# cambyse/po-rrt

Hardware: AMD Instinct MI355X
Metric: RRT node-expansions/sec on map_benchmark.pgm (higher is better)
Workload: dtype f64

## Files before the change

### po_rrt_amd/csrc/porrt_device.hpp

```cpp
#pragma once
#include <hip/hip_runtime.h>
#include <stdint.h>
#include <string>
#include <vector>
#include "../../include/porrt_hip.h"

namespace porrt {

template <int NEV>
struct ScopedEvents {
    hipEvent_t e[NEV];
    ScopedEvents() { for (int i = 0; i < NEV; ++i) e[i] = nullptr; }
    hipError_t create() {
        for (int i = 0; i < NEV; ++i) { const hipError_t r = hipEventCreate(&e[i]); if (r != hipSuccess) return r; }
        return hipSuccess;
    }
    ~ScopedEvents() { for (int i = 0; i < NEV; ++i) if (e[i]) (void)hipEventDestroy(e[i]); }
    ScopedEvents(const ScopedEvents &) = delete;
    ScopedEvents &operator=(const ScopedEvents &) = delete;
};

template <class Launch, class GoingOn>
static int sweep_to_fixpoint(hipStream_t stream, uint32_t *flags, size_t rows, int cur, Launch &&launch, GoingOn &&going_on, const char *who,
                             uint64_t &sweeps, std::string &err) {
// ... 619 lines not shown
        if (m < INF) break;
    }
    if (m == INF && !PTO) m = dist2(rc.nx[0], rc.ny[0], qx, qy);
    return m;
}

__device__ __forceinline__ uint32_t rank_before(const RunConst &rc, uint32_t b, uint32_t vwords, uint32_t k);
__device__ __forceinline__ uint32_t wave_sum(uint32_t v);
__device__ void commit_rrt_sample(const RunConst &rc, uint32_t b, uint32_t vwords, uint32_t k, uint32_t lane, uint32_t stride = 64u, bool lag = false);
constexpr int kRG = 40;
constexpr uint32_t kRegions = kRG * kRG;
constexpr uint32_t kPage = 64;
constexpr uint32_t kOccWords = (kRegions + 63u) / 64u;
typedef double dbl2 __attribute__((ext_vector_type(2)));

__device__ __forceinline__ uint32_t region_of(const RunConst &rc, double x, double y) {
    int cx, cy;
    rep_cell(rc, x, y, kRG, cx, cy);
    return (uint32_t)(cy * kRG + cx);
}

__device__ __forceinline__ double disc_radius(double bound_d2, double qx, double qy) {
    return sqrt(bound_d2) * (1.0 + 1e-9) + 1e-12 * (1.0 + fabs(qx) + fabs(qy));
}

template <class Visit>
__device__ __forceinline__ void scan_disc(const RunConst &rc, uint32_t b, double qx, double qy, double rho, uint32_t N, uint32_t lane, Visit visit,
                                          uint32_t skip_region = 0xFFFFFFFFu, uint32_t share = 0u, uint32_t nshare = 1u) {
    int cx0, cy0, cx1, cy1;
    rep_cell(rc, qx - rho, qy - rho, kRG, cx0, cy0);
    rep_cell(rc, qx + rho, qy + rho, kRG, cx1, cy1);
    const uint32_t x0 = uni((uint32_t)cx0), y0 = uni((uint32_t)cy0);
    const uint32_t w = uni((uint32_t)(cx1 - cx0 + 1)), nreg = w * uni((uint32_t)(cy1 - cy0 + 1));
    if (nreg * 16u > N) {
        auto gx = as_global(rc.nx), gy = as_global(rc.ny);
        for (uint32_t j0 = share * 128u; j0 < N; j0 += nshare * 128u) {
            double x[2], y[2];
#pragma unroll
            for (int u = 0; u < 2; ++u) {
                const uint32_t j = j0 + 64u * u + lane;
                x[u] = gx[j < N ? j : 0u];
                y[u] = gy[j < N ? j : 0u];
            }
#pragma unroll
            for (int u = 0; u < 2; ++u)
                if (j0 + 64u * u < N) visit(x[u], y[u], (int)(j0 + 64u * u + lane), j0 + 64u * u + lane < N);
        }
        return;
    }
    auto gcnt = as_global(rc.rg_cnt) + (b & 1u) * kRegions;
    auto gdir = as_global(rc.rg_dir);
    auto gxy = as_global(reinterpret_cast<const dbl2 *>(rc.pg_xy));
    auto gid = as_global(rc.pg_id);
    for (uint32_t r0 = 0; r0 < nreg; r0 += 64) {
        const uint32_t r = r0 + lane;
        uint32_t reg = 0, cnt = 0;
        if (r < nreg) {
            const uint32_t ry = r / w;
            reg = (y0 + ry) * kRG + x0 + (r - ry * w);
            cnt = reg == skip_region ? 0u : gcnt[reg];
        }
        const uint32_t npg = (uint32_t)__popcll(__ballot(cnt > 0u));
        if (__ballot(cnt >= npg || cnt > kPage) == 0ull && npg > 1u) {
            if (nshare > 1u && r % nshare != share) cnt = 0u;
            uint32_t cmax = cnt;
            for (int off = 32; off > 0; off >>= 1) {
                const uint32_t o = __shfl_xor(cmax, off);
                cmax = o > cmax ? o : cmax;
            }
            cmax = uni(cmax);
            for (uint32_t s0 = 0; s0 < cmax; s0 += 2) {
                dbl2 v[2];
                int id[2];
#pragma unroll
                for (int u = 0; u < 2; ++u) {
                    const uint32_t sl = s0 + u < cnt ? s0 + u : 0u;
                    v[u] = gxy[(size_t)reg * kPage + sl];
                    id[u] = gid[(size_t)reg * kPage + sl];
                }
#pragma unroll
                for (int u = 0; u < 2; ++u)
                    if (s0 + u < cmax) visit(v[u].x, v[u].y, id[u], s0 + u < cnt);
            }
            continue;
        }
        uint32_t page = reg;
        for (uint32_t j = 0;; ++j) {
            unsigned long long m = __ballot(cnt > j * kPage);
            if (!m) break;
            if (nshare > 1u) m = __ballot(cnt > j * kPage && (r + j) % nshare == share);
            if (j && cnt > j * kPage) page = gdir[(size_t)reg * rc.rg_maxp + j];
            while (m) {
                uint32_t pg[2], pc[2];
#pragma unroll
                for (int u = 0; u < 2; ++u) {
                    pg[u] = 0; pc[u] = 0;
                    if (m) {
                        const uint32_t l = (uint32_t)__builtin_ctzll(m);
                        m &= m - 1;
                        pg[u] = (uint32_t)__builtin_amdgcn_readlane((int)page, (int)l);
                        const uint32_t c = (uint32_t)__builtin_amdgcn_readlane((int)cnt, (int)l) - j * kPage;
                        pc[u] = c < kPage ? c : kPage;
                    }
                }
                dbl2 v[2];
                int id[2];
#pragma unroll
                for (int u = 0; u < 2; ++u) {
                    const bool ld = lane < pc[u];
                    v[u] = ld ? gxy[(size_t)pg[u] * kPage + lane] : dbl2{0.0, 0.0};
                    id[u] = ld ? gid[(size_t)pg[u] * kPage + lane] : -1;
                }
#pragma unroll
                for (int u = 0; u < 2; ++u)
                    if (pc[u]) visit(v[u].x, v[u].y, id[u], lane < pc[u]);
            }
        }
    }
}

template <bool PTO>
__device__ __forceinline__ void near_sample(const RunConst &rc, uint32_t b, uint32_t i0, uint32_t vwords, uint32_t k, uint32_t lane) {
    const uint32_t N = uni(as_global(rc.n_at)[b]);
    const double sqx = uni_d(as_global(rc.sx)[i0 + k]), sqy = uni_d(as_global(rc.sy)[i0 + k]);
    uint32_t world = 0;
    if (PTO) world = uni(as_global(rc.sworld)[i0 + k]);
    const double INF = __longlong_as_double(0x7FF0000000000000ll);
// ... 550 lines not shown
    GlobalList L;
    L.cid = as_global((const int *)rc.cand_id) + cand_off(rc, b, k);
    L.cxy = as_global(reinterpret_cast<const dbl2 *>(rc.cand_xy)) + cand_off(rc, b, k);
    L.cval = as_global(rc.cand_val) + cand_val_off(rc, b, k);
    L.gdA = as_global((const double *)rc.distA);
    return L;
}
#ifndef PORRT_LDS_HITS
#define PORRT_LDS_HITS 80
#endif
constexpr uint32_t kLdsHits = PORRT_LDS_HITS;
static_assert(kLdsHits % 2u == 0u, "kLdsHits");
constexpr uint32_t kHitBytes = kLdsHits * (4u + 8u + 8u + 8u);
struct LdsHits {
    static constexpr bool kCompact = true;
    int *hid;
    double *hx, *hy, *hd;
    GPTR(int) out_id;
    GPTR(double) out_val;
    GPTR(uint32_t) out_cnt;
    uint32_t out_cap;
    __device__ __forceinline__ int id(uint32_t a) const { return hid[a]; }
    __device__ __forceinline__ void xy(uint32_t a, double &x, double &y) const { x = hx[a]; y = hy[a]; }
    __device__ __forceinline__ double val(uint32_t a) const { return hx[a]; }
    __device__ __forceinline__ void set_val(uint32_t a, double v) const { hx[a] = v; }
    __device__ __forceinline__ void set_dA(uint32_t, double) const {}
    __device__ __forceinline__ double dA(uint32_t a, int) const { return hd[a]; }
};
struct MemHits {
    static constexpr bool kCompact = true;
    GPTR(int) sid;
    GPTR(dbl2) sxy;
    GPTR(double) sd;
    GPTR(int) out_id;
    GPTR(double) out_val;
    GPTR(uint32_t) out_cnt;
    uint32_t out_cap;
    __device__ __forceinline__ int id(uint32_t a) const { return sid[a]; }
    __device__ __forceinline__ void xy(uint32_t a, double &x, double &y) const { const dbl2 v = sxy[a]; x = v.x; y = v.y; }
    __device__ __forceinline__ double val(uint32_t a) const { return sxy[a].x; }
    __device__ __forceinline__ void set_val(uint32_t a, double v) const { sxy[a].x = v; }
    __device__ __forceinline__ void set_dA(uint32_t, double) const {}
    __device__ __forceinline__ double dA(uint32_t a, int) const { return sd[a]; }
};

struct NoNearestSearch { __device__ int operator()() const { return 0; } };
template <class TeamT, class ListT, class Grid, class NNF = NoNearestSearch>
__device__ void connect_rrt_sample(const RunConst &rc, const TeamT &tm, const ListT &L, const Grid &grid, uint32_t b, uint32_t k, uint32_t id,
                                   double px, double py, uint32_t cnt, uint32_t &err, const uint32_t *clone_ids = nullptr, uint32_t n_clone = 0,
                                   int clr_known = -1, NNF nearest_search = NNF(), uint32_t swap = 0) {
// ... 238 lines not shown
    }
    PORRT_TACC_S(rc, 6);
    auto gdB = as_global(reinterpret_cast<unsigned long long *>(swap ? rc.distA : rc.distB));
    if constexpr (ListT::kCompact) {
        {
            uint32_t n_out = 0;
            for (uint32_t a0 = 0; a0 < cnt; a0 += TS) {
                const uint32_t a = a0 + tl;
                double via = -1.0;
                int j = -1;
                if (a < cnt) {
                    const double cost = a0 == 0 ? cost0 : L.val(a);
                    j = a0 == 0 ? j0 : L.id(a);
                    if (nvalid != 0 && cost >= 0.0 && j != best) {
                        const double v = dnew + cost;
                        if (v < (a0 == 0 ? dA0 : L.dA(a, j))) { g_atomic_min(gdB + j, f64_bits(v)); via = v; }
                    }
                }
                const unsigned long long hm = tm.ballot(via >= 0.0);
                const uint32_t pos = n_out + (uint32_t)__popcll(hm & ((1ull << tm.sub()) - 1ull));
                if (via >= 0.0) {
                    if (pos < L.out_cap) { L.out_id[pos] = j; L.out_val[pos] = via; }
                    else err |= ERR_CAND_OVERFLOW;
                }
                n_out += (uint32_t)__popcll(hm);
            }
            if (tl == 0) *L.out_cnt = n_out;
        }
        PORRT_TACC_S(rc, 7);
        return;
    } else {
// ... 1587 lines not shown
```

### po_rrt_amd/csrc/porrt_engine.hip

```cpp
#include "../../include/porrt_hip.h"
#include "porrt_host.hpp"
#include "porrt_device.hpp"
#include "porrt_group.hpp"
#include "porrt_belief.hpp"
#include "porrt_dp.hpp"
#include "porrt_prm.hpp"
#include "porrt_edges.hpp"
#include "porrt_refine.hpp"
#include "porrt_refine_batch.hpp"
#include "porrt_reparent.hpp"
#include "porrt_qmdp.hpp"
#include "porrt_policy_graph.hpp"
#include "porrt_join.hpp"
#include "porrt_mm_recipe.hpp"

#include <algorithm>
#include <functional>
#include <chrono>
#include <cmath>
#include <cstdio>
#include <cstring>
#include <string>
#include <system_error>
#include <mutex>
// ... 1089 lines not shown
    const uint64_t Nmax = n_iter_max + 2;
    const uint64_t steps_max = n_iter_max / K + 4;
    const uint32_t vwords = (K + 63) / 64;
    const uint32_t Kpad = vwords * 64;
    const uint32_t cand_cap = (uint32_t)std::min<uint64_t>(std::max<uint32_t>(opt_cand_cap, 64), Nmax);
    const uint64_t pend_cap = n_iter_max + 2, pool_cap = tie_pool_ids ? tie_pool_ids : std::max<uint64_t>(1u << 20, tie_pool_mult * n_iter_max);
    {
        double t0 = now_s();
        HIPCHK(d_nx.reserve(Nmax)); HIPCHK(d_ny.reserve(Nmax)); HIPCHK(d_distA.reserve(Nmax)); HIPCHK(d_distB.reserve(Nmax));
        HIPCHK(d_parent.reserve(Nmax)); HIPCHK(d_reachA.reserve(Nmax)); HIPCHK(d_reachB.reserve(Nmax));
        HIPCHK(d_vid.reserve(Nmax)); HIPCHK(d_finalflag.reserve(Nmax + 8)); HIPCHK(d_finalmask.reserve(Nmax));
        HIPCHK(d_nat.reserve(steps_max + 2)); HIPCHK(d_validmask.reserve((steps_max + 2) * vwords));
        HIPCHK(d_sx.reserve(n_iter_max + 1)); HIPCHK(d_sy.reserve(n_iter_max + 1)); HIPCHK(d_sworld.reserve(n_iter_max + 1));
        HIPCHK(d_qx.reserve(2 * Kpad)); HIPCHK(d_qy.reserve(2 * Kpad)); HIPCHK(d_qnn.reserve(2 * Kpad)); HIPCHK(d_qvid.reserve(2 * Kpad));
        const uint64_t rg_maxp = Nmax / kPage + 2, pg_cap = 2ull * kRegions + Nmax / kPage + 8;
        HIPCHK(d_rgcnt.reserve(2 * kRegions)); HIPCHK(d_rgocc.reserve(2 * kOccWords)); HIPCHK(d_rgdir.reserve((size_t)kRegions * rg_maxp));
        HIPCHK(d_pgxy.reserve(2 * (size_t)pg_cap * kPage)); HIPCHK(d_pgid.reserve((size_t)pg_cap * kPage)); HIPCHK(d_pgd.reserve((size_t)pg_cap * kPage)); HIPCHK(d_slotof.reserve(Nmax));
        HIPCHK(d_candcnt.reserve(3 * (size_t)K)); HIPCHK(d_kdbox.reserve(Nmax)); HIPCHK(d_kdlosers.reserve(kClaimMax)); HIPCHK(d_bcscratch.reserve(8 * Nmax + 4096)); HIPCHK(d_bcout.reserve(1)); HIPCHK(d_bccursor.reserve(1)); HIPCHK(d_locbox.reserve(2 * (8 * (size_t)K + 4096))); HIPCHK(d_kdhint.reserve((size_t)kHG * kHG));
        HIPCHK(d_loccur.reserve(2 * (8 * (size_t)K + 4096))); HIPCHK(d_locdcur.reserve(2 * (8 * (size_t)K + 4096))); HIPCHK(d_locgex.reserve(2 * (8 * (size_t)K + 4096))); HIPCHK(d_locflags.reserve(2 * (8 * (size_t)K + 4096)));
        HIPCHK(d_gsnap.reserve((steps_max + 4) * 4)); HIPCHK(d_pendoff.reserve(pend_cap)); HIPCHK(d_pendn.reserve(pend_cap)); HIPCHK(d_pendcur.reserve(pend_cap));
        HIPCHK(d_pendstate.reserve(pend_cap)); HIPCHK(d_pendnew.reserve(pend_cap)); HIPCHK(d_pendpool.reserve(pool_cap)); HIPCHK(d_kdsurv.reserve(Nmax)); HIPCHK(d_gndx.reserve(Nmax)); HIPCHK(d_gndy.reserve(Nmax)); HIPCHK(d_gndbox.reserve(Nmax));
        HIPCHK(d_kqx.reserve((steps_max + 2) * Kpad)); HIPCHK(d_kqy.reserve((steps_max + 2) * Kpad)); HIPCHK(d_kqvid.reserve((steps_max + 2) * Kpad)); { const size_t np = (opt_pipeline == 4 && stage != 1 && K <= 1024) ? 3u : 2u; HIPCHK(d_candid.reserve(np * (size_t)K * cand_cap)); HIPCHK(d_candxy.reserve(2 * np * (size_t)K * cand_cap)); HIPCHK(d_candval.reserve((np == 3u ? 3u : 1u) * (size_t)K * cand_cap)); }
        HIPCHK(d_gid.reserve(Nmax));
        HIPCHK(d_perm.reserve((steps_max + 2) * Kpad)); HIPCHK(d_ssx.reserve((steps_max + 2) * Kpad)); HIPCHK(d_ssy.reserve((steps_max + 2) * Kpad));
        HIPCHK(d_bqx.reserve(Kpad)); HIPCHK(d_bqy.reserve(Kpad)); HIPCHK(d_bqk.reserve(Kpad)); HIPCHK(d_t2at.reserve(steps_max + 4));
        HIPCHK(d_rep.reserve(kRepInts));
        HIPCHK(d_sched_i0.reserve(steps_max + 4)); HIPCHK(d_sched_nb.reserve(steps_max + 4));
        HIPCHK(d_kdrec.reserve(Nmax)); HIPCHK(d_gx.reserve(Nmax + 16)); HIPCHK(d_gy.reserve(Nmax + 16)); HIPCHK(d_kdup.reserve(Nmax)); HIPCHK(d_kddepth.reserve(Nmax)); HIPCHK(d_kdgexit.reserve(Nmax));
        HIPCHK(d_radT2.reserve(Nmax + 8));
        HIPCHK(d_cnt.reserve(1)); HIPCHK(d_rc.reserve(1)); HIPCHK(d_jump.reserve(1));
        if (mode == PORRT_MODE_PTO) {
            const uint64_t ecap = std::min<uint64_t>(Nmax * edge_per_node + 4096, 1ull << 31);
            HIPCHK(d_efrom.reserve(ecap)); HIPCHK(d_eto.reserve(ecap)); HIPCHK(d_etv.reserve(ecap));
        }
        if (has_grid) HIPCHK(d_cls.reserve(cls_bytes(W, H)));
        if (has_inj) HIPCHK(d_inj.reserve(inj_xy.size() + 2));
        int r = layout_buffers();
// ... 3742 lines not shown
```

### po_rrt_amd/csrc/porrt_group.hpp

```cpp
#pragma once
#include "porrt_device.hpp"
#include "porrt_span.hpp"

namespace porrt {


template <int GL, int R, bool WITHD, class Visit>
__device__ __forceinline__ void gscan_disc(const RunConst &rc, uint32_t b, const GTeam<GL> &tm, double qx, double qy, double rho, uint32_t N, Visit visit,
                                           uint32_t skip_region = 0xFFFFFFFFu) {
    const uint32_t gl = tm.gl;
    int cx0, cy0, cx1, cy1;
    rep_cell(rc, qx - rho, qy - rho, kRG, cx0, cy0);
    rep_cell(rc, qx + rho, qy + rho, kRG, cx1, cy1);
    const uint32_t x0 = (uint32_t)cx0, y0 = (uint32_t)cy0;
    const uint32_t w = (uint32_t)(cx1 - cx0 + 1), nreg = w * (uint32_t)(cy1 - cy0 + 1);
    constexpr int U = (int)kPage / GL;
    if (nreg * 16u > N) {
        auto gx = as_global(rc.nx), gy = as_global(rc.ny), gdA = as_global(rc.distA);
        for (uint32_t j0 = 0; j0 < N; j0 += (uint32_t)(U * GL)) {
            double x[U], y[U], d[U];
#pragma unroll
            for (int u = 0; u < U; ++u) {
                const uint32_t j = j0 + (uint32_t)(GL * u) + gl;
                x[u] = gx[j < N ? j : 0u];
                y[u] = gy[j < N ? j : 0u];
                d[u] = WITHD ? gdA[j < N ? j : 0u] : 0.0;
            }
#pragma unroll
            for (int u = 0; u < U; ++u)
                if (j0 + (uint32_t)(GL * u) < N) visit(x[u], y[u], d[u], (int)(j0 + (uint32_t)(GL * u) + gl), j0 + (uint32_t)(GL * u) + gl < N);
        }
        return;
    }
    auto gcnt = as_global(rc.rg_cnt) + (b & 1u) * kRegions;
    auto gdir = as_global(rc.rg_dir);
    auto gxy = as_global(reinterpret_cast<const dbl2 *>(rc.pg_xy));
    auto gid = as_global(rc.pg_id);
    auto gpd = as_global(rc.pg_d);
    for (uint32_t r0 = 0; r0 < nreg; r0 += (uint32_t)GL) {
        const uint32_t r = r0 + gl;
        uint32_t reg = 0, cnt = 0;
        if (r < nreg) {
            const uint32_t ry = r / w;
            reg = (y0 + ry) * kRG + x0 + (r - ry * w);
            cnt = reg == skip_region ? 0u : gcnt[reg];
        }
        uint32_t page = reg;
        for (uint32_t lvl = 0;; ++lvl) {
            const uint32_t have = cnt > lvl * kPage ? cnt - lvl * kPage : 0u;
            unsigned long long m = tm.ballot(have > 0u);
            if (!m) break;
            uint32_t page_next = 0;
            if (have > kPage) page_next = gdir[(size_t)reg * rc.rg_maxp + lvl + 1u];
// ... 7 lines not shown
                        m &= m - 1;
                        pg[q] = tm.shfl(page, l);
                        const uint32_t h = tm.shfl(have, l);
                        pc[q] = h < kPage ? h : kPage;
                    }
                }
                dbl2 v[R][U];
                double d[R][U];
                int id[R][U];
#pragma unroll
                for (int q = 0; q < R; ++q)
#pragma unroll
                    for (int u = 0; u < U; ++u) {
                        const uint32_t sl = (uint32_t)(u * GL) + gl;
                        const bool ld = sl < pc[q];
                        v[q][u] = ld ? gxy[(size_t)pg[q] * kPage + sl] : dbl2{0.0, 0.0};
                        id[q][u] = ld ? gid[(size_t)pg[q] * kPage + sl] : -1;
                        d[q][u] = (WITHD && ld) ? gpd[(size_t)pg[q] * kPage + sl] : 0.0;
                    }
#pragma unroll
                for (int q = 0; q < R; ++q)
#pragma unroll
                    for (int u = 0; u < U; ++u)
                        if ((uint32_t)(u * GL) < pc[q]) visit(v[q][u].x, v[q][u].y, d[q][u], id[q][u], (uint32_t)(u * GL) + gl < pc[q]);
            }
            page = page_next;
        }
    }
}

__device__ __forceinline__ void xcd_swizzle(uint32_t &bx, uint32_t &by) {
    const uint32_t gx = gridDim.x, Q = gridDim.y;
    if (Q & 7u) return;
    const uint32_t L = by * gx + bx, slot = L >> 3;
// ... 85 lines not shown
            }
            m = tm.shfl(d2, 0);
        }
        if (m < INF) break;
    }
    if (m == INF) m = dist2(as_global(rc.nx)[0], as_global(rc.ny)[0], qx, qy);
    return m;
}

#ifndef PORRT_REG_PAGES
#define PORRT_REG_PAGES 1
#endif
template <int GL, class Visit>
__device__ __forceinline__ void gscan_region(const RunConst &rc, const GTeam<GL> &tm, uint32_t reg, uint32_t cnt, Visit visit) {
    auto gdir = as_global(rc.rg_dir);
    auto gxy = as_global(reinterpret_cast<const dbl2 *>(rc.pg_xy));
    auto gid = as_global(rc.pg_id);
    constexpr int U = (int)kPage / GL, RP = PORRT_REG_PAGES;
    const uint32_t npages = (cnt + kPage - 1u) / kPage;
    for (uint32_t j0 = 0; j0 < npages; j0 += (uint32_t)RP) {
        uint32_t page[RP], pc[RP];
#pragma unroll
        for (int q = 0; q < RP; ++q) {
            const uint32_t j = j0 + (uint32_t)q;
            page[q] = 0; pc[q] = 0;
            if (j < npages) {
                page[q] = j ? gdir[(size_t)reg * rc.rg_maxp + j] : reg;
                pc[q] = cnt - j * kPage < kPage ? cnt - j * kPage : kPage;
            }
        }
        dbl2 v[RP][U];
        int id[RP][U];
#pragma unroll
        for (int q = 0; q < RP; ++q)
#pragma unroll
            for (int u = 0; u < U; ++u) {
                const uint32_t sl = (uint32_t)(u * GL) + tm.gl;
                const bool ld = sl < pc[q];
                v[q][u] = ld ? gxy[(size_t)page[q] * kPage + sl] : dbl2{0.0, 0.0};
                id[q][u] = ld ? gid[(size_t)page[q] * kPage + sl] : -1;
            }
#pragma unroll
        for (int q = 0; q < RP; ++q)
#pragma unroll
            for (int u = 0; u < U; ++u)
                if ((uint32_t)(u * GL) < pc[q]) visit(v[q][u].x, v[q][u].y, id[q][u], (uint32_t)(u * GL) + tm.gl < pc[q]);
    }
}

__device__ __forceinline__ double region_gap2(const RunConst &rc, double qx, double qy, int cx, int cy, double wx, double wy) {
    const double INF = __longlong_as_double(0x7FF0000000000000ll);
    const double xlo = cx == 0 ? -INF : rc.bx0 + (double)cx * wx, xhi = cx == kRG - 1 ? INF : rc.bx0 + (double)(cx + 1) * wx;
    const double ylo = cy == 0 ? -INF : rc.by0 + (double)cy * wy, yhi = cy == kRG - 1 ? INF : rc.by0 + (double)(cy + 1) * wy;
    double gx = qx < xlo ? xlo - qx : (qx > xhi ? qx - xhi : 0.0), gy = qy < ylo ? ylo - qy : (qy > yhi ? qy - yhi : 0.0);
    const double eps = 1e-9 * (1.0 + fabs(qx) + fabs(qy));
    gx = gx > eps ? gx - eps : 0.0;
// ... 169 lines not shown
#pragma unroll
        for (uint32_t u = 0; u < kSpanPer; ++u) {
            const uint32_t t = tid * kSpanPer + u, k = k0 + t;
            const uint32_t stored = k < limit ? as_global(rc.cand_cnt)[cand_cnt_at(rc, cb, k)] : 0u;
            c[u] = span_count(stored, cap, span_valid(words, t), k, limit);
            s += c[u];
        }
        uint32_t incl = s;
#pragma unroll
        for (uint32_t off = 1; off < 64u; off <<= 1) {
            const uint32_t v = (uint32_t)__shfl_up((int)incl, off);
            if (tid >= off) incl += v;
        }
        span_prefix_lane(s_prefix, tid, c, incl - s);
    }
    auto gdA = as_global(rc.distA);
    auto gpd = as_global(rc.pg_d);
    auto gso = as_global(rc.slot_of);
    for (uint32_t t = tid; t < kSpan; t += T)
        if (k0 + t < limit && span_valid(words, t)) {
            const uint32_t id = base + span_rank_in(words, t);
            gpd[gso[id]] = gdA[id];
        }
    __syncthreads();
    const uint32_t total = s_prefix[kSpan];
    auto gcid = as_global(rc.cand_id);
    auto gcval = as_global(rc.cand_val);
    auto gdB = as_global(rc.distB);
    constexpr int U = 4;
    for (uint32_t r0 = tid; r0 < total; r0 += T * (uint32_t)U) {
        double via[U], dB[U];
        int j[U], id[U];
#pragma unroll
        for (int u = 0; u < U; ++u) {
            const uint32_t r = r0 + (uint32_t)u * T;
            via[u] = -1.0; j[u] = 0; id[u] = 0;
            if (r < total) {
                const uint32_t t = span_find(s_prefix, r), a = r - s_prefix[t];
                via[u] = gcval[cand_val_off(rc, cb, k0 + t) + a];
                j[u] = gcid[cand_off(rc, cb, k0 + t) + a];
                id[u] = (int)(base + span_rank_in(words, t));
            }
        }
#pragma unroll
        for (int u = 0; u < U; ++u) dB[u] = via[u] >= 0.0 ? gdB[j[u]] : 0.0;
#pragma unroll
        for (int u = 0; u < U; ++u) {
            if (!(via[u] >= 0.0) || f64_bits(via[u]) != f64_bits(dB[u])) continue;
            auto gpar = as_global(rc.parent) + j[u];
            int old = *gpar;
            while (old < N || id[u] < old) {
                int expect = old;
                if (__hip_atomic_compare_exchange_strong(gpar, &expect, id[u], __ATOMIC_RELAXED, __ATOMIC_RELAXED, __HIP_MEMORY_SCOPE_AGENT)) break;
                old = expect;
            }
            gdA[j[u]] = via[u];
            gpd[gso[j[u]]] = via[u];
        }
    }
}

#ifndef PORRT_NN2_WAVES
#define PORRT_NN2_WAVES 5
#endif
template <int GL, int WV = 4>
__global__ __launch_bounds__(WV * 64) __attribute__((amdgpu_waves_per_eu(PORRT_NN2_WAVES, 8))) void k_nn2(const RunConst *__restrict__ rcp, uint32_t b, uint32_t i0, uint32_t nb, uint32_t vwords, uint32_t cb,
                                             uint32_t cnb, uint32_t cflat) {
    static_assert(GL == 16 || GL == 32 || GL == 64, "group size");
    constexpr uint32_t SPB = (uint32_t)WV * 64u / GL;
    uint32_t bx = blockIdx.x, by = blockIdx.y;
    xcd_swizzle(bx, by);
    const RunConst &rc = rc_const(rcp + by);
// ... 135 lines not shown
    t64.gl = threadIdx.x & 63u;
    t64.base = 0;
    int nn;
    double fx, fy;
    group_nn<64>(rc, b, t64, N, px, py, nn, fx, fy);
    return nn;
}

__device__ __forceinline__ void list_scan_wave(const RunConst &rc, uint32_t b, uint32_t N, double T2, uint32_t kh, double pxh, double pyh, uint32_t lane,
                                               uint32_t &err) {
    auto cid = as_global(rc.cand_id) + cand_off(rc, b, kh);
    auto cxy = as_global(reinterpret_cast<dbl2 *>(rc.cand_xy)) + cand_off(rc, b, kh);
    const uint32_t cap = rc.cand_cap;
    uint32_t tot = 0;
    bool over = false;
    scan_disc(rc, b, pxh, pyh, disc_radius(T2, pxh, pyh), uni(N), lane, [&](double x, double y, int jd, bool ok) {
        const bool in = ok && dist2(x, y, pxh, pyh) <= T2;
        const unsigned long long hm = __ballot(in);
        const uint32_t pos = tot + (uint32_t)__popcll(hm & ((1ull << lane) - 1ull));
        if (in) {
            if (pos < cap) {
                cid[pos] = jd;
                dbl2 v;
                v.x = x; v.y = y;
                cxy[pos] = v;
            } else {
                over = true;
            }
        }
        tot += (uint32_t)__popcll(hm);
    });
    if (lane == 0) as_global(rc.cand_cnt)[cand_cnt_at(rc, b, kh)] = tot;
    if (over) err |= (uint32_t)ERR_CAND_OVERFLOW;
}

__device__ __forceinline__ void list_scan_waves(const RunConst &rc, uint32_t b, uint32_t N, double T2, uint32_t kh, double pxh, double pyh, uint32_t lane,
                                                uint32_t wv, uint32_t *tot, uint32_t &err) {
    auto cid = as_global(rc.cand_id) + cand_off(rc, b, kh);
    auto cxy = as_global(reinterpret_cast<dbl2 *>(rc.cand_xy)) + cand_off(rc, b, kh);
    const uint32_t cap = rc.cand_cap;
    bool over = false;
    scan_disc(rc, b, pxh, pyh, disc_radius(T2, pxh, pyh), uni(N), lane, [&](double x, double y, int jd, bool ok) {
        const bool in = ok && dist2(x, y, pxh, pyh) <= T2;
        const unsigned long long hm = __ballot(in);
        if (!hm) return;
        uint32_t base = 0;
        if (lane == 0) base = atomicAdd(tot, (uint32_t)__popcll(hm));
        const uint32_t pos = uni(base) + (uint32_t)__popcll(hm & ((1ull << lane) - 1ull));
        if (in) {
            if (pos < cap) {
                cid[pos] = jd;
                dbl2 v;
                v.x = x; v.y = y;
                cxy[pos] = v;
            } else {
                over = true;
            }
// ... 50 lines not shown
        }
        __syncthreads();
        hc = cand_count(rc, b, kh);
    }
    TableGrid grid;
    grid.p = rc.cls; grid.W = rc.W;
    Team<kConnectWaves> tmh;
    tmh.scr_d = s_d; tmh.scr_i = s_i; tmh.wave = wv; tmh.lane = lane;
    connect_rrt_sample(rc, tmh, global_list(rc, b, kh), grid, b, kh, idh, pxh, pyh, hc, err, s_cid + 1, n - 1u, -1,
                       [&]() { return wave_nn(rc, b, N, pxh, pyh); });
    if (err) atomicOr(&rc.cnt->err, err);
}

__device__ __forceinline__ MemHits mem_hits(const RunConst &rc, uint32_t b, uint32_t k) {
    MemHits M;
    M.sid = as_global(rc.cand_id) + cand_off(rc, b, k);
    M.sxy = as_global(reinterpret_cast<dbl2 *>(rc.cand_xy)) + cand_off(rc, b, k);
    M.sd = as_global(rc.cand_val) + cand_val_off(rc, b, k);
    M.out_id = M.sid;
    M.out_val = M.sd;
    M.out_cnt = as_global(rc.cand_cnt) + cand_cnt_at(rc, b, k);
    M.out_cap = rc.cand_cap;
    return M;
}

template <int GL>
__device__ __attribute__((noinline)) void heavy_sample_wave(const RunConst &rc_arg, uint32_t b, uint32_t N, uint32_t kh, uint32_t idh, uint32_t toth, int clrh,
                                                            double pxh, double pyh, uint8_t *wb, uint32_t &err) {
    const RunConst &rc = rc_const(rc_arg);
    const uint32_t lane = threadIdx.x & 63u;
    constexpr uint32_t kWaveHits = (64u / (uint32_t)GL) * (kLdsHits * (uint32_t)(GL / 16));
    Team<1> tw;
    tw.scr_d = nullptr; tw.scr_i = nullptr; tw.wave = 0; tw.lane = lane;
    TableGrid grid;
    grid.p = rc.cls; grid.W = rc.W;
    const uint32_t cap = rc.cand_cap;
    const MemHits Mh = mem_hits(rc, b, kh);
    PORRT_T0();
    if (toth <= kWaveHits) {
        LdsHits Wl;
        Wl.hx = reinterpret_cast<double *>(wb);
        Wl.hy = Wl.hx + kWaveHits;
        Wl.hd = Wl.hy + kWaveHits;
        Wl.hid = reinterpret_cast<int *>(Wl.hd + kWaveHits);
        Wl.out_id = Mh.out_id; Wl.out_val = Mh.out_val; Wl.out_cnt = Mh.out_cnt; Wl.out_cap = Mh.out_cap;
        for (uint32_t a0 = 0; a0 < toth; a0 += 256u) {
            int jd[4];
            dbl2 v[4];
            double d[4];
#pragma unroll
            for (uint32_t u = 0; u < 4u; ++u) {
                const uint32_t a = a0 + u * 64u + lane;
                jd[u] = a < toth ? Mh.sid[a] : 0;
                v[u] = a < toth ? Mh.sxy[a] : dbl2{0.0, 0.0};
                d[u] = a < toth ? Mh.sd[a] : 0.0;
            }
#pragma unroll
            for (uint32_t u = 0; u < 4u; ++u) {
                const uint32_t a = a0 + u * 64u + lane;
                if (a < toth) { Wl.hid[a] = jd[u]; Wl.hx[a] = v[u].x; Wl.hy[a] = v[u].y; Wl.hd[a] = d[u]; }
            }
        }
        __builtin_amdgcn_wave_barrier();
        PORRT_TACC_H(rc, 0);
        connect_rrt_sample(rc, tw, Wl, grid, b, kh, idh, pxh, pyh, toth, err, nullptr, 0, clrh, [&]() { return wave_nn(rc, b, N, pxh, pyh); });
        __builtin_amdgcn_wave_barrier();
        PORRT_TACC_H(rc, 3);
    } else {
        connect_rrt_sample(rc, tw, Mh, grid, b, kh, idh, pxh, pyh, toth < cap ? toth : cap, err, nullptr, 0, clrh,
                           [&]() { return wave_nn(rc, b, N, pxh, pyh); });
    }
}

#ifndef PORRT_CONN2_WAVES
#define PORRT_CONN2_WAVES 4
#endif
template <int GL>
__device__ __forceinline__ void conn2_wave(const RunConst &rc, uint32_t b, uint32_t vwords, uint32_t N, double T2, uint32_t k, double px, double py, uint8_t *wl) {
    const uint32_t lane = threadIdx.x & 63u;
    GTeam<GL> tm;
    tm.gl = threadIdx.x % GL;
    tm.base = lane - tm.gl;
    const bool act = k != 0xFFFFu;
    uint32_t err = 0;
    PORRT_T0();
    uint32_t id = 0, tot = 0;
    int clr_b = 0;
    bool heavy = false;
    const uint32_t cap = rc.cand_cap;
    TableGrid grid;
    grid.p = rc.cls; grid.W = rc.W;
    if (act) {
        id = N + rank_before_lanes(rc, b, vwords, k, tm.gl, (uint32_t)GL);
        if (rc.has_grid) {
            uint32_t bi, bj;
            to_pixel(rc, px, py, bi, bj);
            if (bi < rc.H && bj < rc.W) clr_b = as_global(rc.clr)[bi * rc.W + bj];
        }
        constexpr uint32_t kHits = kLdsHits * (uint32_t)(GL / 16);
        uint8_t *hb = wl + (lane / (uint32_t)GL) * (kHits * 28u);
        LdsHits L;
        L.hx = reinterpret_cast<double *>(hb);
        L.hy = L.hx + kHits;
        L.hd = L.hy + kHits;
        L.hid = reinterpret_cast<int *>(L.hd + kHits);
        const MemHits M = mem_hits(rc, b, k);
        L.out_id = M.out_id; L.out_val = M.out_val; L.out_cnt = M.out_cnt; L.out_cap = M.out_cap;
        PORRT_TACC_B(rc, 0);
        gscan_disc<GL, 1, true>(rc, b, tm, px, py, disc_radius(T2, px, py), N, [&](double x, double y, double dA, int jd, bool ok) {
            const bool in = ok && dist2(x, y, px, py) <= T2;
            const unsigned long long hm = tm.ballot(in);
            const uint32_t pos = tot + (uint32_t)__popcll(hm & ((1ull << tm.gl) - 1ull));
            if (in) {
                if (pos < kHits) { L.hid[pos] = jd; L.hx[pos] = x; L.hy[pos] = y; L.hd[pos] = dA; }
                else if (pos < cap) { M.sid[pos] = jd; dbl2 v; v.x = x; v.y = y; M.sxy[pos] = v; M.sd[pos] = dA; }
                else err |= (uint32_t)ERR_CAND_OVERFLOW;
            }
            tot += (uint32_t)__popcll(hm);
        });
        __builtin_amdgcn_wave_barrier();
// ... 102 lines not shown
```

Measured before the change: 339.7 million.

## Use buffer loads and 32-bit offsets for page and hit-list accesses

Page reads (xy, id, d) in the disc scans now go through AMD raw buffer resource loads. Masked-off lanes read an out-of-range slot, so the hardware returns zero instead of the code selecting a value. Hit lists and several global accesses now use 32-bit byte offsets, and LDS pointers carry an explicit address space. The aim is to cut 64-bit address arithmetic, flat-address overhead and select instructions on a hot, memory-bound path. In exchange, host-side checks cap arrays below 4 GiB, and signal fences are added that may limit how the compiler schedules these loads.

```diff
diff --git a/po_rrt_amd/csrc/porrt_device.hpp b/po_rrt_amd/csrc/porrt_device.hpp
--- a/po_rrt_amd/csrc/porrt_device.hpp
+++ b/po_rrt_amd/csrc/porrt_device.hpp
@@ -657,6 +657,59 @@
 constexpr uint32_t kOccWords = (kRegions + 63u) / 64u;
 typedef double dbl2 __attribute__((ext_vector_type(2)));
 
+#ifndef PORRT_PAGE_LOADS
+#define PORRT_PAGE_LOADS 1
+#endif
+constexpr uint32_t kNoSlot = 0x0FFFFFFFu;
+struct PageBuf {
+    __amdgpu_buffer_rsrc_t xy, id, d;
+};
+__device__ __forceinline__ __amdgpu_buffer_rsrc_t buf_of(const void *p, uint32_t bytes) {
+    return __builtin_amdgcn_make_buffer_rsrc(const_cast<void *>(p), (short)0, (int)bytes, 0x00020000);
+}
+__device__ __forceinline__ PageBuf page_buf(const RunConst &rc) {
+    const uint32_t slots = rc.pg_cap * kPage;
+    PageBuf pb;
+    pb.xy = buf_of(rc.pg_xy, slots * 16u);
+    pb.id = buf_of(rc.pg_id, slots * 4u);
+    pb.d = buf_of(rc.pg_d, slots * 8u);
+    return pb;
+}
+typedef uint32_t u32x2 __attribute__((ext_vector_type(2)));
+typedef uint32_t u32x4 __attribute__((ext_vector_type(4)));
+__device__ __forceinline__ dbl2 page_xy(const PageBuf &pb, uint32_t slot) {
+    return __builtin_bit_cast(dbl2, (u32x4)__builtin_amdgcn_raw_buffer_load_b128(pb.xy, (int)(slot << 4), 0, 0));
+}
+__device__ __forceinline__ int page_id(const PageBuf &pb, uint32_t slot) {
+    return (int)__builtin_amdgcn_raw_buffer_load_b32(pb.id, (int)(slot << 2), 0, 0);
+}
+__device__ __forceinline__ double page_d(const PageBuf &pb, uint32_t slot) {
+    return __builtin_bit_cast(double, (u32x2)__builtin_amdgcn_raw_buffer_load_b64(pb.d, (int)(slot << 3), 0, 0));
+}
+template <class T>
+__device__ __forceinline__ T g_at(const T *base, uint32_t byte_off) {
+    return *(GPTR(const T))((GPTR(const char))(uintptr_t)base + byte_off);
+}
+template <class T>
+__device__ __forceinline__ GPTR(T) g_ptr(T *base, uint32_t byte_off) {
+    return (GPTR(T))((GPTR(char))(uintptr_t)base + byte_off);
+}
+template <class T>
+struct Row32 {
+    T *base;
+    uint32_t off;
+    __device__ __forceinline__ T __attribute__((address_space(1))) &operator[](uint32_t i) const {
+        return *(GPTR(T))((GPTR(char))(uintptr_t)base + (off + i) * (uint32_t)sizeof(T));
+    }
+};
+#if PORRT_PAGE_LOADS
+template <class T> using HitRow = Row32<T>;
+template <class T> using LdsPtr = T __attribute__((address_space(3))) *;
+#else
+template <class T> using HitRow = T __attribute__((address_space(1))) *;
+template <class T> using LdsPtr = T *;
+#endif
+
 __device__ __forceinline__ uint32_t region_of(const RunConst &rc, double x, double y) {
     int cx, cy;
     rep_cell(rc, x, y, kRG, cx, cy);
@@ -667,7 +720,7 @@
     return sqrt(bound_d2) * (1.0 + 1e-9) + 1e-12 * (1.0 + fabs(qx) + fabs(qy));
 }
 
-template <class Visit>
+template <bool BUF = false, class Visit>
 __device__ __forceinline__ void scan_disc(const RunConst &rc, uint32_t b, double qx, double qy, double rho, uint32_t N, uint32_t lane, Visit visit,
                                           uint32_t skip_region = 0xFFFFFFFFu, uint32_t share = 0u, uint32_t nshare = 1u) {
     int cx0, cy0, cx1, cy1;
@@ -676,14 +729,19 @@
     const uint32_t x0 = uni((uint32_t)cx0), y0 = uni((uint32_t)cy0);
     const uint32_t w = uni((uint32_t)(cx1 - cx0 + 1)), nreg = w * uni((uint32_t)(cy1 - cy0 + 1));
     if (nreg * 16u > N) {
-        auto gx = as_global(rc.nx), gy = as_global(rc.ny);
+        [[maybe_unused]] auto gx = as_global(rc.nx), gy = as_global(rc.ny);
         for (uint32_t j0 = share * 128u; j0 < N; j0 += nshare * 128u) {
             double x[2], y[2];
 #pragma unroll
             for (int u = 0; u < 2; ++u) {
                 const uint32_t j = j0 + 64u * u + lane;
-                x[u] = gx[j < N ? j : 0u];
-                y[u] = gy[j < N ? j : 0u];
+                if constexpr (BUF) {
+                    x[u] = g_at(rc.nx, (j < N ? j : 0u) * 8u);
+                    y[u] = g_at(rc.ny, (j < N ? j : 0u) * 8u);
+                } else {
+                    x[u] = gx[j < N ? j : 0u];
+                    y[u] = gy[j < N ? j : 0u];
+                }
             }
 #pragma unroll
             for (int u = 0; u < 2; ++u)
@@ -693,8 +751,10 @@
     }
     auto gcnt = as_global(rc.rg_cnt) + (b & 1u) * kRegions;
     auto gdir = as_global(rc.rg_dir);
-    auto gxy = as_global(reinterpret_cast<const dbl2 *>(rc.pg_xy));
-    auto gid = as_global(rc.pg_id);
+    [[maybe_unused]] auto gxy = as_global(reinterpret_cast<const dbl2 *>(rc.pg_xy));
+    [[maybe_unused]] auto gid = as_global(rc.pg_id);
+    [[maybe_unused]] PageBuf pb;
+    if constexpr (BUF) pb = page_buf(rc);
     for (uint32_t r0 = 0; r0 < nreg; r0 += 64) {
         const uint32_t r = r0 + lane;
         uint32_t reg = 0, cnt = 0;
@@ -717,10 +777,17 @@
                 int id[2];
 #pragma unroll
                 for (int u = 0; u < 2; ++u) {
-                    const uint32_t sl = s0 + u < cnt ? s0 + u : 0u;
-                    v[u] = gxy[(size_t)reg * kPage + sl];
-                    id[u] = gid[(size_t)reg * kPage + sl];
+                    if constexpr (BUF) {
+                        const uint32_t at = s0 + u < cnt ? reg * kPage + s0 + u : kNoSlot;
+                        v[u] = page_xy(pb, at);
+                        id[u] = page_id(pb, at);
+                    } else {
+                        const uint32_t sl = s0 + u < cnt ? s0 + u : 0u;
+                        v[u] = gxy[(size_t)reg * kPage + sl];
+                        id[u] = gid[(size_t)reg * kPage + sl];
+                    }
                 }
+                if constexpr (BUF) __atomic_signal_fence(__ATOMIC_SEQ_CST);
 #pragma unroll
                 for (int u = 0; u < 2; ++u)
                     if (s0 + u < cmax) visit(v[u].x, v[u].y, id[u], s0 + u < cnt);
@@ -751,9 +818,16 @@
 #pragma unroll
                 for (int u = 0; u < 2; ++u) {
                     const bool ld = lane < pc[u];
-                    v[u] = ld ? gxy[(size_t)pg[u] * kPage + lane] : dbl2{0.0, 0.0};
-                    id[u] = ld ? gid[(size_t)pg[u] * kPage + lane] : -1;
+                    if constexpr (BUF) {
+                        const uint32_t at = ld ? pg[u] * kPage + lane : kNoSlot;
+                        v[u] = page_xy(pb, at);
+                        id[u] = page_id(pb, at);
+                    } else {
+                        v[u] = ld ? gxy[(size_t)pg[u] * kPage + lane] : dbl2{0.0, 0.0};
+                        id[u] = ld ? gid[(size_t)pg[u] * kPage + lane] : -1;
+                    }
                 }
+                if constexpr (BUF) __atomic_signal_fence(__ATOMIC_SEQ_CST);
 #pragma unroll
                 for (int u = 0; u < 2; ++u)
                     if (pc[u]) visit(v[u].x, v[u].y, id[u], lane < pc[u]);
@@ -1334,10 +1408,10 @@
 constexpr uint32_t kHitBytes = kLdsHits * (4u + 8u + 8u + 8u);
 struct LdsHits {
     static constexpr bool kCompact = true;
-    int *hid;
-    double *hx, *hy, *hd;
-    GPTR(int) out_id;
-    GPTR(double) out_val;
+    LdsPtr<int> hid;
+    LdsPtr<double> hx, hy, hd;
+    HitRow<int> out_id;
+    HitRow<double> out_val;
     GPTR(uint32_t) out_cnt;
     uint32_t out_cap;
     __device__ __forceinline__ int id(uint32_t a) const { return hid[a]; }
@@ -1349,11 +1423,11 @@
 };
 struct MemHits {
     static constexpr bool kCompact = true;
-    GPTR(int) sid;
-    GPTR(dbl2) sxy;
-    GPTR(double) sd;
-    GPTR(int) out_id;
-    GPTR(double) out_val;
+    HitRow<int> sid;
+    HitRow<dbl2> sxy;
+    HitRow<double> sd;
+    HitRow<int> out_id;
+    HitRow<double> out_val;
     GPTR(uint32_t) out_cnt;
     uint32_t out_cap;
     __device__ __forceinline__ int id(uint32_t a) const { return sid[a]; }
@@ -1622,7 +1696,14 @@
                     j = a0 == 0 ? j0 : L.id(a);
                     if (nvalid != 0 && cost >= 0.0 && j != best) {
                         const double v = dnew + cost;
+#if PORRT_PAGE_LOADS
+                        if (v < (a0 == 0 ? dA0 : L.dA(a, j))) {
+                            g_atomic_min(g_ptr(reinterpret_cast<unsigned long long *>(swap ? rc.distA : rc.distB), (uint32_t)j * 8u), f64_bits(v));
+                            via = v;
+                        }
+#else
                         if (v < (a0 == 0 ? dA0 : L.dA(a, j))) { g_atomic_min(gdB + j, f64_bits(v)); via = v; }
+#endif
                     }
                 }
                 const unsigned long long hm = tm.ballot(via >= 0.0);
diff --git a/po_rrt_amd/csrc/porrt_engine.hip b/po_rrt_amd/csrc/porrt_engine.hip
--- a/po_rrt_amd/csrc/porrt_engine.hip
+++ b/po_rrt_amd/csrc/porrt_engine.hip
@@ -1127,13 +1127,16 @@
         HIPCHK(d_sx.reserve(n_iter_max + 1)); HIPCHK(d_sy.reserve(n_iter_max + 1)); HIPCHK(d_sworld.reserve(n_iter_max + 1));
         HIPCHK(d_qx.reserve(2 * Kpad)); HIPCHK(d_qy.reserve(2 * Kpad)); HIPCHK(d_qnn.reserve(2 * Kpad)); HIPCHK(d_qvid.reserve(2 * Kpad));
         const uint64_t rg_maxp = Nmax / kPage + 2, pg_cap = 2ull * kRegions + Nmax / kPage + 8;
+        if (16ull * pg_cap * kPage >= (1ull << 32)) { set_err("n_iter_max too large: a page array of 4 GiB or more"); return PORRT_ERR_CAPACITY; }
         HIPCHK(d_rgcnt.reserve(2 * kRegions)); HIPCHK(d_rgocc.reserve(2 * kOccWords)); HIPCHK(d_rgdir.reserve((size_t)kRegions * rg_maxp));
         HIPCHK(d_pgxy.reserve(2 * (size_t)pg_cap * kPage)); HIPCHK(d_pgid.reserve((size_t)pg_cap * kPage)); HIPCHK(d_pgd.reserve((size_t)pg_cap * kPage)); HIPCHK(d_slotof.reserve(Nmax));
         HIPCHK(d_candcnt.reserve(3 * (size_t)K)); HIPCHK(d_kdbox.reserve(Nmax)); HIPCHK(d_kdlosers.reserve(kClaimMax)); HIPCHK(d_bcscratch.reserve(8 * Nmax + 4096)); HIPCHK(d_bcout.reserve(1)); HIPCHK(d_bccursor.reserve(1)); HIPCHK(d_locbox.reserve(2 * (8 * (size_t)K + 4096))); HIPCHK(d_kdhint.reserve((size_t)kHG * kHG));
         HIPCHK(d_loccur.reserve(2 * (8 * (size_t)K + 4096))); HIPCHK(d_locdcur.reserve(2 * (8 * (size_t)K + 4096))); HIPCHK(d_locgex.reserve(2 * (8 * (size_t)K + 4096))); HIPCHK(d_locflags.reserve(2 * (8 * (size_t)K + 4096)));
         HIPCHK(d_gsnap.reserve((steps_max + 4) * 4)); HIPCHK(d_pendoff.reserve(pend_cap)); HIPCHK(d_pendn.reserve(pend_cap)); HIPCHK(d_pendcur.reserve(pend_cap));
         HIPCHK(d_pendstate.reserve(pend_cap)); HIPCHK(d_pendnew.reserve(pend_cap)); HIPCHK(d_pendpool.reserve(pool_cap)); HIPCHK(d_kdsurv.reserve(Nmax)); HIPCHK(d_gndx.reserve(Nmax)); HIPCHK(d_gndy.reserve(Nmax)); HIPCHK(d_gndbox.reserve(Nmax));
-        HIPCHK(d_kqx.reserve((steps_max + 2) * Kpad)); HIPCHK(d_kqy.reserve((steps_max + 2) * Kpad)); HIPCHK(d_kqvid.reserve((steps_max + 2) * Kpad)); { const size_t np = (opt_pipeline == 4 && stage != 1 && K <= 1024) ? 3u : 2u; HIPCHK(d_candid.reserve(np * (size_t)K * cand_cap)); HIPCHK(d_candxy.reserve(2 * np * (size_t)K * cand_cap)); HIPCHK(d_candval.reserve((np == 3u ? 3u : 1u) * (size_t)K * cand_cap)); }
+        HIPCHK(d_kqx.reserve((steps_max + 2) * Kpad)); HIPCHK(d_kqy.reserve((steps_max + 2) * Kpad)); HIPCHK(d_kqvid.reserve((steps_max + 2) * Kpad)); { const size_t np = (opt_pipeline == 4 && stage != 1 && K <= 1024) ? 3u : 2u;
+          if (16ull * np * K * cand_cap >= (1ull << 32)) { set_err("cand_cap too large: a neighbour-list array of 4 GiB or more"); return PORRT_ERR_CAPACITY; }
+          HIPCHK(d_candid.reserve(np * (size_t)K * cand_cap)); HIPCHK(d_candxy.reserve(2 * np * (size_t)K * cand_cap)); HIPCHK(d_candval.reserve((np == 3u ? 3u : 1u) * (size_t)K * cand_cap)); }
         HIPCHK(d_gid.reserve(Nmax));
         HIPCHK(d_perm.reserve((steps_max + 2) * Kpad)); HIPCHK(d_ssx.reserve((steps_max + 2) * Kpad)); HIPCHK(d_ssy.reserve((steps_max + 2) * Kpad));
         HIPCHK(d_bqx.reserve(Kpad)); HIPCHK(d_bqy.reserve(Kpad)); HIPCHK(d_bqk.reserve(Kpad)); HIPCHK(d_t2at.reserve(steps_max + 4));
diff --git a/po_rrt_amd/csrc/porrt_group.hpp b/po_rrt_amd/csrc/porrt_group.hpp
--- a/po_rrt_amd/csrc/porrt_group.hpp
+++ b/po_rrt_amd/csrc/porrt_group.hpp
@@ -16,15 +16,24 @@
     const uint32_t w = (uint32_t)(cx1 - cx0 + 1), nreg = w * (uint32_t)(cy1 - cy0 + 1);
     constexpr int U = (int)kPage / GL;
     if (nreg * 16u > N) {
+#if !PORRT_PAGE_LOADS
         auto gx = as_global(rc.nx), gy = as_global(rc.ny), gdA = as_global(rc.distA);
+#endif
         for (uint32_t j0 = 0; j0 < N; j0 += (uint32_t)(U * GL)) {
             double x[U], y[U], d[U];
 #pragma unroll
             for (int u = 0; u < U; ++u) {
                 const uint32_t j = j0 + (uint32_t)(GL * u) + gl;
+#if PORRT_PAGE_LOADS
+                const uint32_t o = (j < N ? j : 0u) * 8u;
+                x[u] = g_at(rc.nx, o);
+                y[u] = g_at(rc.ny, o);
+                d[u] = WITHD ? g_at(rc.distA, o) : 0.0;
+#else
                 x[u] = gx[j < N ? j : 0u];
                 y[u] = gy[j < N ? j : 0u];
                 d[u] = WITHD ? gdA[j < N ? j : 0u] : 0.0;
+#endif
             }
 #pragma unroll
             for (int u = 0; u < U; ++u)
@@ -34,9 +43,13 @@
     }
     auto gcnt = as_global(rc.rg_cnt) + (b & 1u) * kRegions;
     auto gdir = as_global(rc.rg_dir);
+#if PORRT_PAGE_LOADS
+    const PageBuf pb = page_buf(rc);
+#else
     auto gxy = as_global(reinterpret_cast<const dbl2 *>(rc.pg_xy));
     auto gid = as_global(rc.pg_id);
     auto gpd = as_global(rc.pg_d);
+#endif
     for (uint32_t r0 = 0; r0 < nreg; r0 += (uint32_t)GL) {
         const uint32_t r = r0 + gl;
         uint32_t reg = 0, cnt = 0;
@@ -74,10 +87,20 @@
                     for (int u = 0; u < U; ++u) {
                         const uint32_t sl = (uint32_t)(u * GL) + gl;
                         const bool ld = sl < pc[q];
+#if PORRT_PAGE_LOADS
+                        const uint32_t at = ld ? pg[q] * kPage + sl : kNoSlot;
+                        v[q][u] = page_xy(pb, at);
+                        id[q][u] = page_id(pb, at);
+                        d[q][u] = WITHD ? page_d(pb, at) : 0.0;
+#else
                         v[q][u] = ld ? gxy[(size_t)pg[q] * kPage + sl] : dbl2{0.0, 0.0};
                         id[q][u] = ld ? gid[(size_t)pg[q] * kPage + sl] : -1;
                         d[q][u] = (WITHD && ld) ? gpd[(size_t)pg[q] * kPage + sl] : 0.0;
+#endif
                     }
+#if PORRT_PAGE_LOADS
+                __atomic_signal_fence(__ATOMIC_SEQ_CST);
+#endif
 #pragma unroll
                 for (int q = 0; q < R; ++q)
 #pragma unroll
@@ -193,8 +216,12 @@
 template <int GL, class Visit>
 __device__ __forceinline__ void gscan_region(const RunConst &rc, const GTeam<GL> &tm, uint32_t reg, uint32_t cnt, Visit visit) {
     auto gdir = as_global(rc.rg_dir);
+#if PORRT_PAGE_LOADS
+    const PageBuf pb = page_buf(rc);
+#else
     auto gxy = as_global(reinterpret_cast<const dbl2 *>(rc.pg_xy));
     auto gid = as_global(rc.pg_id);
+#endif
     constexpr int U = (int)kPage / GL, RP = PORRT_REG_PAGES;
     const uint32_t npages = (cnt + kPage - 1u) / kPage;
     for (uint32_t j0 = 0; j0 < npages; j0 += (uint32_t)RP) {
@@ -216,9 +243,18 @@
             for (int u = 0; u < U; ++u) {
                 const uint32_t sl = (uint32_t)(u * GL) + tm.gl;
                 const bool ld = sl < pc[q];
+#if PORRT_PAGE_LOADS
+                const uint32_t at = ld ? page[q] * kPage + sl : kNoSlot;
+                v[q][u] = page_xy(pb, at);
+                id[q][u] = page_id(pb, at);
+#else
                 v[q][u] = ld ? gxy[(size_t)page[q] * kPage + sl] : dbl2{0.0, 0.0};
                 id[q][u] = ld ? gid[(size_t)page[q] * kPage + sl] : -1;
-            }
+#endif
+            }
+#if PORRT_PAGE_LOADS
+        __atomic_signal_fence(__ATOMIC_SEQ_CST);
+#endif
 #pragma unroll
         for (int q = 0; q < RP; ++q)
 #pragma unroll
@@ -418,19 +454,27 @@
         }
         span_prefix_lane(s_prefix, tid, c, incl - s);
     }
+#if !PORRT_PAGE_LOADS
     auto gdA = as_global(rc.distA);
     auto gpd = as_global(rc.pg_d);
     auto gso = as_global(rc.slot_of);
+#endif
     for (uint32_t t = tid; t < kSpan; t += T)
         if (k0 + t < limit && span_valid(words, t)) {
             const uint32_t id = base + span_rank_in(words, t);
+#if PORRT_PAGE_LOADS
+            *g_ptr(rc.pg_d, g_at(rc.slot_of, id * 4u) * 8u) = g_at(rc.distA, id * 8u);
+#else
             gpd[gso[id]] = gdA[id];
+#endif
         }
     __syncthreads();
     const uint32_t total = s_prefix[kSpan];
+#if !PORRT_PAGE_LOADS
     auto gcid = as_global(rc.cand_id);
     auto gcval = as_global(rc.cand_val);
     auto gdB = as_global(rc.distB);
+#endif
     constexpr int U = 4;
     for (uint32_t r0 = tid; r0 < total; r0 += T * (uint32_t)U) {
         double via[U], dB[U];
@@ -441,25 +485,43 @@
             via[u] = -1.0; j[u] = 0; id[u] = 0;
             if (r < total) {
                 const uint32_t t = span_find(s_prefix, r), a = r - s_prefix[t];
+#if PORRT_PAGE_LOADS
+                via[u] = g_at(rc.cand_val, ((uint32_t)cand_val_off(rc, cb, k0 + t) + a) * 8u);
+                j[u] = g_at(rc.cand_id, ((uint32_t)cand_off(rc, cb, k0 + t) + a) * 4u);
+#else
                 via[u] = gcval[cand_val_off(rc, cb, k0 + t) + a];
                 j[u] = gcid[cand_off(rc, cb, k0 + t) + a];
+#endif
                 id[u] = (int)(base + span_rank_in(words, t));
             }
         }
 #pragma unroll
+#if PORRT_PAGE_LOADS
+        for (int u = 0; u < U; ++u) dB[u] = via[u] >= 0.0 ? g_at(rc.distB, (uint32_t)j[u] * 8u) : 0.0;
+#else
         for (int u = 0; u < U; ++u) dB[u] = via[u] >= 0.0 ? gdB[j[u]] : 0.0;
+#endif
 #pragma unroll
         for (int u = 0; u < U; ++u) {
             if (!(via[u] >= 0.0) || f64_bits(via[u]) != f64_bits(dB[u])) continue;
+#if PORRT_PAGE_LOADS
+            auto gpar = g_ptr(rc.parent, (uint32_t)j[u] * 4u);
+#else
             auto gpar = as_global(rc.parent) + j[u];
+#endif
             int old = *gpar;
             while (old < N || id[u] < old) {
                 int expect = old;
                 if (__hip_atomic_compare_exchange_strong(gpar, &expect, id[u], __ATOMIC_RELAXED, __ATOMIC_RELAXED, __HIP_MEMORY_SCOPE_AGENT)) break;
                 old = expect;
             }
+#if PORRT_PAGE_LOADS
+            *g_ptr(rc.distA, (uint32_t)j[u] * 8u) = via[u];
+            *g_ptr(rc.pg_d, g_at(rc.slot_of, (uint32_t)j[u] * 4u) * 8u) = via[u];
+#else
             gdA[j[u]] = via[u];
             gpd[gso[j[u]]] = via[u];
+#endif
         }
     }
 }
@@ -625,7 +687,7 @@
     const uint32_t cap = rc.cand_cap;
     uint32_t tot = 0;
     bool over = false;
-    scan_disc(rc, b, pxh, pyh, disc_radius(T2, pxh, pyh), uni(N), lane, [&](double x, double y, int jd, bool ok) {
+    scan_disc<PORRT_PAGE_LOADS != 0>(rc, b, pxh, pyh, disc_radius(T2, pxh, pyh), uni(N), lane, [&](double x, double y, int jd, bool ok) {
         const bool in = ok && dist2(x, y, pxh, pyh) <= T2;
         const unsigned long long hm = __ballot(in);
         const uint32_t pos = tot + (uint32_t)__popcll(hm & ((1ull << lane) - 1ull));
@@ -651,7 +713,7 @@
     auto cxy = as_global(reinterpret_cast<dbl2 *>(rc.cand_xy)) + cand_off(rc, b, kh);
     const uint32_t cap = rc.cand_cap;
     bool over = false;
-    scan_disc(rc, b, pxh, pyh, disc_radius(T2, pxh, pyh), uni(N), lane, [&](double x, double y, int jd, bool ok) {
+    scan_disc<PORRT_PAGE_LOADS != 0>(rc, b, pxh, pyh, disc_radius(T2, pxh, pyh), uni(N), lane, [&](double x, double y, int jd, bool ok) {
         const bool in = ok && dist2(x, y, pxh, pyh) <= T2;
         const unsigned long long hm = __ballot(in);
         if (!hm) return;
@@ -732,9 +794,15 @@
 
 __device__ __forceinline__ MemHits mem_hits(const RunConst &rc, uint32_t b, uint32_t k) {
     MemHits M;
+#if PORRT_PAGE_LOADS
+    M.sid = {rc.cand_id, (uint32_t)cand_off(rc, b, k)};
+    M.sxy = {reinterpret_cast<dbl2 *>(rc.cand_xy), (uint32_t)cand_off(rc, b, k)};
+    M.sd = {rc.cand_val, (uint32_t)cand_val_off(rc, b, k)};
+#else
     M.sid = as_global(rc.cand_id) + cand_off(rc, b, k);
     M.sxy = as_global(reinterpret_cast<dbl2 *>(rc.cand_xy)) + cand_off(rc, b, k);
     M.sd = as_global(rc.cand_val) + cand_val_off(rc, b, k);
+#endif
     M.out_id = M.sid;
     M.out_val = M.sd;
     M.out_cnt = as_global(rc.cand_cnt) + cand_cnt_at(rc, b, k);
@@ -744,8 +812,13 @@
 
 template <int GL>
 __device__ __attribute__((noinline)) void heavy_sample_wave(const RunConst &rc_arg, uint32_t b, uint32_t N, uint32_t kh, uint32_t idh, uint32_t toth, int clrh,
-                                                            double pxh, double pyh, uint8_t *wb, uint32_t &err) {
+                                                            double pxh, double pyh, uint8_t *wb, uint32_t &err_out) {
     const RunConst &rc = rc_const(rc_arg);
+#if PORRT_PAGE_LOADS
+    uint32_t err = 0;
+#else
+    uint32_t &err = err_out;
+#endif
     const uint32_t lane = threadIdx.x & 63u;
     constexpr uint32_t kWaveHits = (64u / (uint32_t)GL) * (kLdsHits * (uint32_t)(GL / 16));
     Team<1> tw;
@@ -757,10 +830,10 @@
     PORRT_T0();
     if (toth <= kWaveHits) {
         LdsHits Wl;
-        Wl.hx = reinterpret_cast<double *>(wb);
+        Wl.hx = (LdsPtr<double>)wb;
         Wl.hy = Wl.hx + kWaveHits;
         Wl.hd = Wl.hy + kWaveHits;
-        Wl.hid = reinterpret_cast<int *>(Wl.hd + kWaveHits);
+        Wl.hid = (LdsPtr<int>)(Wl.hd + kWaveHits);
         Wl.out_id = Mh.out_id; Wl.out_val = Mh.out_val; Wl.out_cnt = Mh.out_cnt; Wl.out_cap = Mh.out_cap;
         for (uint32_t a0 = 0; a0 < toth; a0 += 256u) {
             int jd[4];
@@ -788,6 +861,9 @@
         connect_rrt_sample(rc, tw, Mh, grid, b, kh, idh, pxh, pyh, toth < cap ? toth : cap, err, nullptr, 0, clrh,
                            [&]() { return wave_nn(rc, b, N, pxh, pyh); });
     }
+#if PORRT_PAGE_LOADS
+    if (err) err_out |= err;
+#endif
 }
 
 #ifndef PORRT_CONN2_WAVES
@@ -818,10 +894,10 @@
         constexpr uint32_t kHits = kLdsHits * (uint32_t)(GL / 16);
         uint8_t *hb = wl + (lane / (uint32_t)GL) * (kHits * 28u);
         LdsHits L;
-        L.hx = reinterpret_cast<double *>(hb);
+        L.hx = (LdsPtr<double>)hb;
         L.hy = L.hx + kHits;
         L.hd = L.hy + kHits;
-        L.hid = reinterpret_cast<int *>(L.hd + kHits);
+        L.hid = (LdsPtr<int>)(L.hd + kHits);
         const MemHits M = mem_hits(rc, b, k);
         L.out_id = M.out_id; L.out_val = M.out_val; L.out_cnt = M.out_cnt; L.out_cap = M.out_cap;
         PORRT_TACC_B(rc, 0);
```

After: 352.2 million (median of 6 runs). +3.7%, better.
